# cvxpy/cvxpylayers

Measured on NVIDIA B200. Metric: QP problems/sec fwd+bwd (batch=4096, n=100, m=200, zero+nonneg cones), higher is better.
Workload: dtype f64

## Files before the change

cvxpylayers_b200/_lib.py:

```python
from __future__ import annotations

import ctypes as C
import os
from pathlib import Path

_PKG = Path(__file__).resolve().parent
LIB_PATH = Path(os.environ["BCONE_LIB"]) if os.environ.get("BCONE_LIB") else _PKG / "libbcone.so"

_i32p = C.POINTER(C.c_int32)
_f64p = C.POINTER(C.c_double)

EXPORTS = [
    "bcone_default_settings", "bcone_create", "bcone_destroy", "bcone_last_error", "bcone_set_boundary", "bcone_set_boundary_quad",
    "bcone_ingest", "bcone_emit", "bcone_ingest_pitched", "bcone_emit_pitched", "bcone_peer_alloc", "bcone_peer_open", "bcone_peer_close",
    "bcone_peer_free", "bcone_copy2d_async", "bcone_rows_from_param", "bcone_param_from_rows", "bcone_gather_cols", "bcone_scatter_cols", "bcone_set_param_maps", "bcone_ingest_params", "bcone_emit_params", "bcone_solve", "bcone_solve_warm", "bcone_solve_cached", "bcone_cache_bytes", "bcone_vjp", "bcone_launch_count", "bcone_fallback_count", "bcone_kernel_info", "bcone_path_info", "bcone_memcpy2d", "bcone_set_profile",
]


class BconeDesc(C.Structure):
    _fields_ = [("n", C.c_int32), ("m", C.c_int32), ("nnzA", C.c_int32), ("nnzP", C.c_int32),
                ("A_indptr", _i32p), ("A_indices", _i32p), ("P_indptr", _i32p), ("P_indices", _i32p),
                ("z", C.c_int32), ("l", C.c_int32), ("nq", C.c_int32), ("ns", C.c_int32),
                ("ep", C.c_int32), ("ed", C.c_int32), ("q", _i32p), ("s", _i32p),
                ("device", C.c_int32), ("max_batch", C.c_int32)]


class BconeSettings(C.Structure):
    _fields_ = [("eps_abs", C.c_double), ("eps_rel", C.c_double), ("eps_infeas", C.c_double),
                ("alpha", C.c_double), ("rho_x", C.c_double), ("scale", C.c_double),
                ("lsqr_atol", C.c_double), ("lsqr_btol", C.c_double), ("lsqr_conlim", C.c_double),
                ("max_iters", C.c_int32), ("normalize", C.c_int32), ("adaptive_scale", C.c_int32),
                ("check_interval", C.c_int32), ("ruiz_passes", C.c_int32), ("lsqr_iter_lim", C.c_int32),
                ("lsqr_precond", C.c_int32), ("adaptive_check", C.c_int32),
                ("acceleration_lookback", C.c_int32), ("acceleration_interval", C.c_int32)]


class EngineUnavailable(RuntimeError):
    """libbcone.so is missing / cannot be loaded. There is deliberately no fallback."""


_lib = None


def load() -> C.CDLL:
    global _lib
    if _lib is not None:
        return _lib
    if not LIB_PATH.exists():
        raise EngineUnavailable(
            f"{LIB_PATH} not found: build it with `python -m cvxpylayers_b200.build` (nvcc, sm_100a). "
            "The engine has no CPU or PyTorch fallback.")
    try:
        lib = C.CDLL(str(LIB_PATH))
    except OSError as e:
        raise EngineUnavailable(f"cannot load {LIB_PATH}: {e}") from e
    vp = C.c_void_p
    lib.bcone_default_settings.argtypes = [C.POINTER(BconeSettings)]
    lib.bcone_default_settings.restype = None
    lib.bcone_create.argtypes = [C.POINTER(BconeDesc), C.POINTER(vp)]
    lib.bcone_create.restype = C.c_int
    lib.bcone_destroy.argtypes = [vp]
    lib.bcone_destroy.restype = None
    lib.bcone_last_error.argtypes = [vp]
    lib.bcone_last_error.restype = C.c_char_p
    lib.bcone_set_boundary.argtypes = [vp, C.c_int32, _i32p, C.c_int32, _i32p]
    lib.bcone_set_boundary.restype = C.c_int
    lib.bcone_set_boundary_quad.argtypes = [vp, C.c_int32, _i32p]
    lib.bcone_set_boundary_quad.restype = C.c_int
    lib.bcone_ingest.argtypes = [vp, C.c_int32] + [vp] * 8
    lib.bcone_ingest.restype = C.c_int
    lib.bcone_emit.argtypes = [vp, C.c_int32] + [vp] * 8
    lib.bcone_emit.restype = C.c_int
    lib.bcone_ingest_pitched.argtypes = [vp, C.c_int32, C.c_int64] + [vp] * 8
    lib.bcone_ingest_pitched.restype = C.c_int
    lib.bcone_emit_pitched.argtypes = [vp, C.c_int32, C.c_int64] + [vp] * 8
    lib.bcone_emit_pitched.restype = C.c_int
    lib.bcone_peer_alloc.argtypes = [C.c_int32, C.c_int64, C.POINTER(vp), vp]
    lib.bcone_peer_alloc.restype = C.c_int
    lib.bcone_peer_open.argtypes = [C.c_int32, vp, C.POINTER(vp)]
    lib.bcone_peer_open.restype = C.c_int
    lib.bcone_peer_close.argtypes = [vp]
    lib.bcone_peer_close.restype = C.c_int
    lib.bcone_peer_free.argtypes = [vp]
    lib.bcone_peer_free.restype = C.c_int
    lib.bcone_copy2d_async.argtypes = [vp, C.c_int64, vp, C.c_int64, C.c_int64, C.c_int64, vp]
    lib.bcone_copy2d_async.restype = C.c_int
    lib.bcone_rows_from_param.argtypes = [vp, C.c_int64, vp, C.c_int32, C.c_int32, C.c_int32, vp, vp]
    lib.bcone_rows_from_param.restype = C.c_int
    lib.bcone_param_from_rows.argtypes = [vp, vp, C.c_int64, vp, C.c_int32, C.c_int32, C.c_int32, vp, vp]
    lib.bcone_param_from_rows.restype = C.c_int
    lib.bcone_gather_cols.argtypes = [vp, C.c_int64, vp, vp, C.c_int32, C.c_int32, C.c_int32, vp, vp]
    lib.bcone_gather_cols.restype = C.c_int
    lib.bcone_scatter_cols.argtypes = [vp, vp, C.c_int64, vp, vp, C.c_int32, C.c_int32, C.c_int32, vp, vp]
    lib.bcone_scatter_cols.restype = C.c_int
    lib.bcone_set_param_maps.argtypes = [vp, C.c_int32] + [_i32p, _i32p, _f64p] * 3
    lib.bcone_set_param_maps.restype = C.c_int
    lib.bcone_ingest_params.argtypes = [vp, C.c_int32] + [vp] * 6
    lib.bcone_ingest_params.restype = C.c_int
    lib.bcone_emit_params.argtypes = [vp, C.c_int32] + [vp] * 6
    lib.bcone_emit_params.restype = C.c_int
    lib.bcone_solve.argtypes = [vp, C.c_int32] + [vp] * 10 + [C.POINTER(BconeSettings), vp]
    lib.bcone_solve.restype = C.c_int
    lib.bcone_solve_warm.argtypes = [vp, C.c_int32] + [vp] * 13 + [C.POINTER(BconeSettings), vp]
    lib.bcone_solve_warm.restype = C.c_int
    lib.bcone_solve_cached.argtypes = [vp, C.c_int32] + [vp] * 13 + [vp, C.c_int32, C.POINTER(BconeSettings), vp]
    lib.bcone_solve_cached.restype = C.c_int
    lib.bcone_cache_bytes.argtypes = [vp, C.c_int32]
    lib.bcone_cache_bytes.restype = C.c_size_t
    lib.bcone_vjp.argtypes = [vp, C.c_int32] + [vp] * 14 + [C.POINTER(BconeSettings), vp]
    lib.bcone_vjp.restype = C.c_int
    lib.bcone_memcpy2d.argtypes = [vp, C.c_int64, vp, C.c_int64, C.c_int64, C.c_int64, C.c_int32, vp]
    lib.bcone_memcpy2d.restype = C.c_int
    lib.bcone_set_profile.argtypes = [vp, C.c_int32, C.POINTER(C.c_uint64)]
    lib.bcone_set_profile.restype = C.c_int
    lib.bcone_launch_count.argtypes = [vp]
    lib.bcone_launch_count.restype = C.c_int64
    lib.bcone_fallback_count.argtypes = [vp, _i32p]
    lib.bcone_fallback_count.restype = C.c_int
    lib.bcone_kernel_info.argtypes = [vp] + [_i32p] * 6
    lib.bcone_kernel_info.restype = C.c_int
    lib.bcone_path_info.argtypes = [vp, _i32p, _i32p]
    lib.bcone_path_info.restype = C.c_int
    _lib = lib
    return lib


def default_settings() -> BconeSettings:
    st = BconeSettings()
    load().bcone_default_settings(C.byref(st))
    return st
```

cvxpylayers_b200/csrc/api.cu:

```cuda
#include <cuda_runtime.h>
#include <algorithm>
#include <cstdio>
#include <cstring>
#include <string>
#include <vector>
#include <cstdlib>
#include "common.cuh"

extern "C" {
size_t bc_fwd_smem_bytes(int n, int m, int nnzA, int threads, int max_psd, int indirect, int ns, int nexp);
size_t bc_fwd_ws_doubles(int n, int m, int with_factor);
cudaError_t bc_fwd_configure(int dense, int indirect, size_t smem, int small_cta);
cudaError_t bc_fwd_occupancy(int dense, int indirect, int threads, size_t smem, int *ctas, int small_cta);
cudaError_t bc_fwd_launch(const FwdArgs *a, int indirect, int grid, int threads, size_t smem, cudaStream_t st, int small_cta);
size_t bc_fwdf_smem_bytes(int n, int m);
int bc_fwdf_threads(void);
size_t bc_fwdf_cache_doubles(int n, int m);
int bc_fwdf_eligible(int n, int m);
cudaError_t bc_fwdf_configure(int n, int m, size_t smem);
cudaError_t bc_fwdf_occupancy(int n, int m, size_t smem, int *ctas);
cudaError_t bc_fwdf_launch(const FwdArgs *a, int grid, size_t smem, cudaStream_t st);
size_t bc_bwd_ws_doubles(int n, int m, int npoly);
size_t bc_bwd_smem_bytes(int n, int m, int npoly, int nnzA, int nnzP_smem, int threads, int max_psd, int psd_total, int nexp, int vec_global);
cudaError_t bc_bwd_configure(int dense, size_t smem, int small_cta);
// ... 557 lines not shown
  CK(cudaSetDevice(h->device), "vjp set device");
  a.ws = nullptr; a.ws_stride = (long long)h->bwd_ws_stride;
  if (h->bwd_vec_global && !h->fast_bwd) {
    Handle::StreamWs *sw = stream_ws(h, st);
    if (!ensure_slab(h, &sw->bwd, nullptr, h->bwd_ws_stride * (size_t)h->num_sms * std::max(h->bwd_ctas, h->bwd_ctas_small))) return fail(h, BCONE_ENOMEM, "cudaMalloc backward workspace");
    a.ws = sw->bwd;
  }
  a.inst_list = nullptr; a.B_dev = nullptr; a.fail_list = nullptr; a.fail_count = nullptr; a.prof = h->prof;
  if (h->block_bwd && stg->lsqr_precond == 2) {
    if (h->fail_cap[slot] < B) {
      int *p = nullptr;
      CK(cudaMalloc((void **)&p, (size_t)B * sizeof(int)), "vjp fail list");
      h->allocs.push_back(p); h->fail_list[slot] = p; h->fail_cap[slot] = B;
    }
    CK(cudaMemsetAsync(ctr + 1, 0, 3 * sizeof(int), st), "vjp counters");
    h->last_block_slot = slot;
    a.fail_list = h->fail_list[slot]; a.fail_count = ctr + 2;
    CK(bc_bwdb_launch(&a, std::min(B, h->num_sms), h->blk_threads, h->blk_smem, st), "vjp launch (block)");
    BwdArgs f = a;
    f.st.lsqr_precond = 1; f.counter = ctr + 3; f.inst_list = h->fail_list[slot]; f.B_dev = ctr + 2;
    f.fail_list = nullptr; f.fail_count = nullptr;
    CK(bc_bwdf_launch(&f, std::min(B, h->num_sms * h->bwd_ctas), h->bwd_threads, h->bwd_smem, st), "vjp launch (fallback)");
    h->launches += 2;
    return BCONE_OK;
  }
  if (a.st.lsqr_precond == 2) a.st.lsqr_precond = 1;
  CK(cudaMemsetAsync(ctr + 1, 0, sizeof(int), st), "vjp counter");
  const int use_small = h->bwd_small && (h->small_mode == 2 || B > h->num_sms * h->bwd_ctas);
  const int grid = std::min(B, h->num_sms * (use_small ? h->bwd_ctas_small : h->bwd_ctas));
  if (h->fast_bwd) CK(bc_bwdf_launch(&a, grid, h->bwd_threads, h->bwd_smem, st), "vjp launch (fast)");
  else CK(bc_bwd_launch(&a, grid, h->bwd_threads, h->bwd_smem, st, use_small), "vjp launch");
  h->launches++;
  return BCONE_OK;
}

extern "C" int bcone_memcpy2d(void *dst, int64_t dpitch, const void *src, int64_t spitch, int64_t width, int64_t height,
                              int32_t to_device, void *stream) {
  cudaError_t e = cudaMemcpy2DAsync(dst, (size_t)dpitch, src, (size_t)spitch, (size_t)width, (size_t)height,
                                    to_device ? cudaMemcpyHostToDevice : cudaMemcpyDeviceToHost, (cudaStream_t)stream);
  if (e != cudaSuccess) { g_create_err = std::string("bcone_memcpy2d: ") + cudaGetErrorString(e); return BCONE_ECUDA; }
  return BCONE_OK;
}

extern "C" int bcone_set_profile(void *handle, int32_t on, uint64_t *out) {
  Handle *h = (Handle *)handle;
  if (!h) return BCONE_EINVAL;
  cudaSetDevice(h->device);
  if (out && h->prof) { cudaDeviceSynchronize(); cudaMemcpy(out, h->prof, 32 * sizeof(uint64_t), cudaMemcpyDeviceToHost); cudaMemset(h->prof, 0, 32 * sizeof(uint64_t)); }
  if (on && !h->prof) { if (cudaMalloc((void **)&h->prof, 32 * sizeof(uint64_t)) != cudaSuccess) return BCONE_ENOMEM; h->allocs.push_back(h->prof); cudaMemset(h->prof, 0, 32 * sizeof(uint64_t)); }
  if (!on) h->prof = nullptr;
  return BCONE_OK;
}

extern "C" int bcone_fallback_count(void *handle, int32_t *out) {
  Handle *h = (Handle *)handle;
  if (!h || !out) return BCONE_EINVAL;
  *out = -1;
  if (h->last_block_slot < 0) return BCONE_OK;
  cudaSetDevice(h->device);
  if (cudaDeviceSynchronize() != cudaSuccess) return BCONE_ECUDA;
  int v = 0;
  if (cudaMemcpy(&v, h->counters + 4 * h->last_block_slot + 2, sizeof(int), cudaMemcpyDeviceToHost) != cudaSuccess) return BCONE_ECUDA;
  *out = v;
  return BCONE_OK;
}

extern "C" int64_t bcone_launch_count(void *handle) { return handle ? ((Handle *)handle)->launches : 0; }

extern "C" int bcone_path_info(void *handle, int32_t *fwd_path, int32_t *bwd_path) {
  Handle *h = (Handle *)handle;
  if (!h) return BCONE_EINVAL;
  if (fwd_path) *fwd_path = h->fast_fwd ? 2 : (h->fwd_indirect ? 1 : (h->fwd_factor_global ? 3 : 0));
  if (bwd_path) *bwd_path = h->block_bwd ? 2 : (h->fast_bwd ? 1 : 0);
  return BCONE_OK;
}

extern "C" int bcone_kernel_info(void *handle, int32_t *ft, int32_t *fs, int32_t *fc, int32_t *bt, int32_t *bs, int32_t *bcx) {
  Handle *h = (Handle *)handle;
  if (!h) return BCONE_EINVAL;
  if (ft) *ft = h->fwd_threads; if (fs) *fs = (int32_t)h->fwd_smem; if (fc) *fc = h->fwd_ctas;
  if (bt) *bt = h->bwd_threads; if (bs) *bs = (int32_t)h->bwd_smem; if (bcx) *bcx = h->bwd_ctas;
  return BCONE_OK;
}
```

cvxpylayers_b200/csrc/common.cuh:

```cuda
#pragma once
#include <cuda_runtime.h>
#include <stdint.h>
#include "../../include/bcone.h"

#define BC_TAU_FACTOR 10.0
#define BC_ZERO_CONE_FACTOR 1000.0
#define BC_MIN_SCALE 1e-4
#define BC_MAX_SCALE 1e4
#define BC_RESCALE_MIN_ITERS 100
#define BC_EQ_MIN 1e-4
#define BC_EQ_MAX 1e4

enum { BC_CZERO = 0, BC_CNONNEG = 1, BC_CSOC = 2, BC_CPSD = 3 };

struct DevStruct {
  int n, m, nnzA, nnzP;
  int z, l, nq, ns;
  int ep, ed, exp_start;
  int dense;
  int ncones;
  int max_psd;
  const int *A_indptr, *A_indices;
  const int *At_colptr, *At_rowidx, *At_perm;
  const int *A_rowof;
// ... 513 lines not shown
}

template <bool SQ = false, class Epi>
__device__ __forceinline__ void csr_rows(const double *__restrict__ vals, const int *__restrict__ indptr,
                                         const int *__restrict__ indices, int nrows,
                                         const double *x, Epi ep) {
  constexpr int G = 4;
  const int g = threadIdx.x % G, grp = threadIdx.x / G, ngrp = blockDim.x / G;
  for (int base = 0; base < nrows; base += ngrp) {
    const int i = base + grp;
    double a = 0;
    if (i < nrows) {
      const int e = __ldg(indptr + i + 1);
      for (int k = __ldg(indptr + i) + g; k < e; k += G) { const double q = vals[k]; a = fma(SQ ? q * q : q, x[__ldg(indices + k)], a); }
    }
    a += __shfl_xor_sync(0xffffffffu, a, 1);
    a += __shfl_xor_sync(0xffffffffu, a, 2);
    if (g == 0 && i < nrows) ep(i, a);
  }
}
template <bool SQ = false, class Epi>
__device__ __forceinline__ void csr_cols(const double *__restrict__ vals, const int *__restrict__ colptr,
                                         const int *__restrict__ rowidx, const int *__restrict__ perm, int ncols,
                                         const double *y, Epi ep) {
  constexpr int G = 4;
  const int g = threadIdx.x % G, grp = threadIdx.x / G, ngrp = blockDim.x / G;
  for (int base = 0; base < ncols; base += ngrp) {
    const int j = base + grp;
    double a = 0;
    if (j < ncols) {
      const int e = __ldg(colptr + j + 1);
      for (int k = __ldg(colptr + j) + g; k < e; k += G) { const double q = vals[__ldg(perm + k)]; a = fma(SQ ? q * q : q, y[__ldg(rowidx + k)], a); }
    }
    a += __shfl_xor_sync(0xffffffffu, a, 1);
    a += __shfl_xor_sync(0xffffffffu, a, 2);
    if (g == 0 && j < ncols) ep(j, a);
  }
}

template <bool DENSE, bool SQ = false, class Epi>
__device__ __forceinline__ void A_mul(const DevStruct &S, const double *Av, const double *x, Epi ep, bool wide = false) {
  if (DENSE && wide) dense_rows2<SQ>(Av, S.m, S.n, x, ep);
  else if (DENSE) matvec_rows<SQ>(Av, DenseLayout{S.n}, S.m, S.n, x, ep);
  else csr_rows<SQ>(Av, S.A_indptr, S.A_indices, S.m, x, ep);
}
template <bool DENSE, bool SQ = false, class Epi>
__device__ __forceinline__ void AT_mul(const DevStruct &S, const double *Av, const double *y, double *part, Epi ep, const ColPlan &plA,
                                       bool wide = false) {
  if (DENSE && wide) dense_cols2<SQ>(Av, S.m, S.n, y, part, ep);
  else if (DENSE) matvec_cols<SQ>(Av, DenseLayout{S.n}, S.m, S.n, y, part, ep, plA);
  else { csr_cols<SQ>(Av, S.At_colptr, S.At_rowidx, S.At_perm, S.n, y, ep); __syncthreads(); }
}

template <bool SQ = false, class Epi>
__device__ __forceinline__ void P_mul(const DevStruct &S, const double *Pv, const double *x, double *part, Epi ep, const ColPlan &plN) {
  const int n = S.n;
  if (S.p_dense) {
    matvec_rows<SQ>(Pv, PackedUpperLayout<false>{n}, n, n, x, ep);
    __syncthreads();
    matvec_cols<SQ>(Pv, PackedUpperLayout<true>{n}, n, n, x, part, ep, plN);
  } else {
    csr_rows<SQ>(Pv, S.P_indptr, S.P_indices, n, x, ep);
    __syncthreads();
    constexpr int G = 4;
    const int g = threadIdx.x % G, grp = threadIdx.x / G, ngrp = blockDim.x / G;
    for (int base = 0; base < n; base += ngrp) {
      const int j = base + grp;
      double a = 0;
      if (j < n) {
        const int e = __ldg(S.Pt_colptr + j + 1);
        for (int k = __ldg(S.Pt_colptr + j) + g; k < e; k += G) {
          const int i = __ldg(S.Pt_rowidx + k);
          if (i != j) { const double q = Pv[__ldg(S.Pt_perm + k)]; a = fma(SQ ? q * q : q, x[i], a); }
        }
      }
      a += __shfl_xor_sync(0xffffffffu, a, 1);
      a += __shfl_xor_sync(0xffffffffu, a, 2);
      if (g == 0 && j < n) ep(j, a);
    }
    __syncthreads();
  }
}

__host__ __device__ __forceinline__ int chol_scratch_doubles(int n) { return 26 * ((n + 3) >> 2) + 2; }
__device__ __forceinline__ double rsqrt_nr(double x) {
  double y;
  asm("rsqrt.approx.ftz.f64 %0, %1;" : "=d"(y) : "d"(x));
  double e = fma(-x * y, y, 1.0);
  y = fma(0.5 * y, e, y);
  e = fma(-x * y, y, 1.0);
  return fma(0.5 * y, e, y);
}
struct Tri4 { double l00, l10, l11, l20, l21, l22, l30, l31, l32, l33, m00, m10, m11, m20, m21, m22, m30, m31, m32, m33; bool pd; };
__device__ __forceinline__ Tri4 tri4_block(const double *K, int r0, int jb) {
  Tri4 q;
  const double *R0 = K + ((r0 * (r0 + 1)) >> 1) + r0;
  const double *R1 = K + (((r0 + 1) * (r0 + 2)) >> 1) + r0, *R2 = K + (((r0 + 2) * (r0 + 3)) >> 1) + r0, *R3 = K + (((r0 + 3) * (r0 + 4)) >> 1) + r0;
  const double d00 = R0[0];
  const double d10 = jb > 1 ? R1[0] : 0.0, d11 = jb > 1 ? R1[1] : 1.0;
  const double d20 = jb > 2 ? R2[0] : 0.0, d21 = jb > 2 ? R2[1] : 0.0, d22 = jb > 2 ? R2[2] : 1.0;
  const double d30 = jb > 3 ? R3[0] : 0.0, d31 = jb > 3 ? R3[1] : 0.0, d32 = jb > 3 ? R3[2] : 0.0, d33 = jb > 3 ? R3[3] : 1.0;
  const double p0 = d00, r0_ = rsqrt_nr(p0);
  q.l00 = p0 * r0_; q.l10 = d10 * r0_; q.l20 = d20 * r0_; q.l30 = d30 * r0_;
  const double p1 = fma(-q.l10, q.l10, d11), r1_ = rsqrt_nr(p1);
  q.l11 = p1 * r1_; q.l21 = fma(-q.l20, q.l10, d21) * r1_; q.l31 = fma(-q.l30, q.l10, d31) * r1_;
  const double p2 = fma(-q.l21, q.l21, fma(-q.l20, q.l20, d22)), r2_ = rsqrt_nr(p2);
  q.l22 = p2 * r2_; q.l32 = fma(-q.l31, q.l21, fma(-q.l30, q.l20, d32)) * r2_;
  const double p3 = fma(-q.l32, q.l32, fma(-q.l31, q.l31, fma(-q.l30, q.l30, d33))), r3_ = rsqrt_nr(p3);
  q.l33 = p3 * r3_;
  q.pd = (p0 > 0) && (p1 > 0) && (p2 > 0) && (p3 > 0);
  q.m00 = r0_; q.m11 = r1_; q.m22 = r2_; q.m33 = r3_;
  q.m10 = -q.l10 * q.m00 * r1_;
  q.m20 = -fma(q.l21, q.m10, q.l20 * q.m00) * r2_; q.m21 = -q.l21 * q.m11 * r2_;
  q.m30 = -fma(q.l32, q.m20, fma(q.l31, q.m10, q.l30 * q.m00)) * r3_;
  q.m31 = -fma(q.l32, q.m21, q.l31 * q.m11) * r3_; q.m32 = -q.l32 * q.m22 * r3_;
  return q;
}
#ifdef BC_CHOLPROF
#define CP_STAMP(k) if (prof && t == 0) { const long long now_ = clock64(); atomicAdd(prof + (k), (unsigned long long)(now_ - tt)); tt = now_; }
#else
#define CP_STAMP(k)
#endif
__device__ inline bool chol_inv_packed(double *K, int n, double *tmp, unsigned long long *prof = nullptr) {
  const int T = blockDim.x, t = threadIdx.x, lane = t & 31, warp = t >> 5, nw = T >> 5;
  const int nblk = (n + 3) >> 2, ld = 4 * nblk;
  double *isd = tmp, *moff = tmp + 4 * nblk, *Tst = tmp + 10 * nblk, *flag = tmp + 26 * nblk;
  long long t0 = 0;
  if (prof && t == 0) t0 = clock64();
#ifdef BC_CHOLPROF
  long long tt = t0;
#endif
  const int fr = lane >> 2, fc = lane & 3;
  auto diag_block = [&](int J0) {
    const int jb = min(4, n - J0);
    const Tri4 q = tri4_block(K, J0, jb);
    __syncwarp();
    if (lane == 0) {
      double *D0 = K + ((J0 * (J0 + 1)) >> 1) + J0;
      D0[0] = q.l00;
      if (jb > 1) { double *D1 = K + (((J0 + 1) * (J0 + 2)) >> 1) + J0; D1[0] = q.l10; D1[1] = q.l11; }
      if (jb > 2) { double *D2 = K + (((J0 + 2) * (J0 + 3)) >> 1) + J0; D2[0] = q.l20; D2[1] = q.l21; D2[2] = q.l22; }
      if (jb > 3) { double *D3 = K + (((J0 + 3) * (J0 + 4)) >> 1) + J0; D3[0] = q.l30; D3[1] = q.l31; D3[2] = q.l32; D3[3] = q.l33; }
      isd[J0] = q.m00; isd[J0 + 1] = q.m11; isd[J0 + 2] = q.m22; isd[J0 + 3] = q.m33;
      double *mo = moff + 6 * (J0 >> 2);
      mo[0] = q.m10; mo[1] = q.m20; mo[2] = q.m21; mo[3] = q.m30; mo[4] = q.m31; mo[5] = q.m32;
      if (!q.pd) *flag = 0.0;
    }
  };
  auto trail_tile = [&](int ta, int tb, int J0, int jb, int R0) {
    const int ra = R0 + 8 * ta + fr, rb = R0 + 8 * tb + fr;
    const double fa = (ra < n && fc < jb) ? -K[((ra * (ra + 1)) >> 1) + J0 + fc] : 0.0;
    const double fb = (rb < n && fc < jb) ? K[((rb * (rb + 1)) >> 1) + J0 + fc] : 0.0;
    const int cc = R0 + 8 * tb + 2 * fc;
    double *pc = K + ((ra * (ra + 1)) >> 1) + cc;
    const bool ok0 = ra < n && cc <= ra, ok1 = ra < n && cc + 1 <= ra;
    double c0 = ok0 ? pc[0] : 0.0, c1 = ok1 ? pc[1] : 0.0;
    dmma884(c0, c1, fa, fb);
    if (ok0) pc[0] = c0;
    if (ok1) pc[1] = c1;
  };
  auto inv_tile = [&](int jt, int I0, int ib) {
    double c0 = 0.0, c1 = 0.0, d0 = 0.0, d1 = 0.0;
    const bool zr = fr < ib;
    const double *zrow = K + (((I0 + (zr ? fr : 0)) * (I0 + (zr ? fr : 0) + 1)) >> 1);
    const int jcol = 8 * jt + fr;
    int k = 8 * jt;
    for (int q = 0; q < 2 && k < I0; q++, k += 4) {
      const int k0 = k + fc;
      const double a0 = zr ? zrow[k0] : 0.0;
      const double b0 = jcol <= k0 ? K[((k0 * (k0 + 1)) >> 1) + jcol] : 0.0;
      if (q == 0) dmma884(c0, c1, a0, b0); else dmma884(d0, d1, a0, b0);
    }
    int k0 = k + fc, o0 = ((k0 * (k0 + 1)) >> 1) + jcol;
    for (; k + 8 <= I0; k += 8) {
      const int o1 = o0 + 4 * k0 + 10;
      const double a0 = zr ? zrow[k0] : 0.0, a1 = zr ? zrow[k0 + 4] : 0.0;
      const double b0 = K[o0], b1 = K[o1];
      dmma884(c0, c1, a0, b0);
      dmma884(d0, d1, a1, b1);
      o0 += 8 * k0 + 36; k0 += 8;
    }
    if (k < I0) {
      const double a0 = zr ? zrow[k0] : 0.0;
      dmma884(c0, c1, a0, K[o0]);
    }
    if (fr < 4) {
      const int col = 8 * jt + 2 * fc;
      Tst[fr * ld + col] = c0 + d0; Tst[fr * ld + col + 1] = c1 + d1;
    }
  };
  auto store_X = [&](int I0) {
    const int ib = min(4, n - I0);
    for (int j = (t + (T >> 1)) % T; j < I0; j += T) {
      K[((I0 * (I0 + 1)) >> 1) + j] = Tst[j];
      if (ib > 1) K[(((I0 + 1) * (I0 + 2)) >> 1) + j] = Tst[ld + j];
      if (ib > 2) K[(((I0 + 2) * (I0 + 3)) >> 1) + j] = Tst[2 * ld + j];
      if (ib > 3) K[(((I0 + 3) * (I0 + 4)) >> 1) + j] = Tst[3 * ld + j];
    }
    if (t == T - 1) {
      const double *mo = moff + 6 * (I0 >> 2);
      double *D0 = K + ((I0 * (I0 + 1)) >> 1) + I0;
      D0[0] = isd[I0];
      if (ib > 1) { double *D1 = K + (((I0 + 1) * (I0 + 2)) >> 1) + I0; D1[0] = mo[0]; D1[1] = isd[I0 + 1]; }
      if (ib > 2) { double *D2 = K + (((I0 + 2) * (I0 + 3)) >> 1) + I0; D2[0] = mo[1]; D2[1] = mo[2]; D2[2] = isd[I0 + 2]; }
      if (ib > 3) { double *D3 = K + (((I0 + 3) * (I0 + 4)) >> 1) + I0; D3[0] = mo[3]; D3[1] = mo[4]; D3[2] = mo[5]; D3[3] = isd[I0 + 3]; }
    }
  };
  if (warp == 0) {
    if (lane == 0) *flag = 1.0;
    __syncwarp();
    diag_block(0);
  }
  __syncthreads();
  for (int J0 = 0; J0 < n; J0 += 4) {
    const int jb = min(4, n - J0), R0 = J0 + jb;
    if (*flag == 0.0) return false;
    if (J0 > 0) store_X(J0 - 4);
    const int tz = (t + T - (T >> 2)) % T;
    if (R0 + t < n || tz < J0) {
      const double *mo = moff + 6 * (J0 >> 2);
      const double m00 = isd[J0], m11 = isd[J0 + 1], m22 = isd[J0 + 2], m33 = isd[J0 + 3];
      const double m10 = mo[0], m20 = mo[1], m21 = mo[2], m30 = mo[3], m31 = mo[4], m32 = mo[5];
      for (int i = R0 + t; i < n; i += T) {
        double *row = K + ((i * (i + 1)) >> 1) + J0;
        const double a0 = row[0], a1 = jb > 1 ? row[1] : 0.0, a2 = jb > 2 ? row[2] : 0.0, a3 = jb > 3 ? row[3] : 0.0;
        row[0] = a0 * m00;
        if (jb > 1) row[1] = fma(a1, m11, a0 * m10);
        if (jb > 2) row[2] = fma(a2, m22, fma(a1, m21, a0 * m20));
        if (jb > 3) row[3] = fma(a3, m33, fma(a2, m32, fma(a1, m31, a0 * m30)));
      }
      double *L0 = K + ((J0 * (J0 + 1)) >> 1), *L1 = K + (((J0 + 1) * (J0 + 2)) >> 1), *L2 = K + (((J0 + 2) * (J0 + 3)) >> 1),
             *L3 = K + (((J0 + 3) * (J0 + 4)) >> 1);
      for (int i = tz; i < J0; i += T) {
        const double a0 = L0[i], a1 = jb > 1 ? L1[i] : 0.0, a2 = jb > 2 ? L2[i] : 0.0, a3 = jb > 3 ? L3[i] : 0.0;
        L0[i] = -(m00 * a0);
        if (jb > 1) L1[i] = -fma(m11, a1, m10 * a0);
        if (jb > 2) L2[i] = -fma(m22, a2, fma(m21, a1, m20 * a0));
        if (jb > 3) L3[i] = -fma(m33, a3, fma(m32, a2, fma(m31, a1, m30 * a0)));
      }
    }
    CP_STAMP(17);
    __syncthreads();
    CP_STAMP(18);
    {
      const int ntl = R0 < n ? (n - R0 + 7) >> 3 : 0, ntile = (ntl * (ntl + 1)) >> 1;
      const int ntj = (J0 + 7) >> 3;
      if (warp == 0 && ntile > 0) {
        trail_tile(0, 0, J0, jb, R0);
        __syncwarp();
        diag_block(R0);
      }
      if (warp > 0 || nw == 1) {
        const int W = nw > 1 ? nw - 1 : 1, w0 = nw > 1 ? warp - 1 : 0;
        const int nwork = ntj + (ntile > 0 ? ntile - 1 : 0);
        int ta = 0, tb = 0, e_cur = 0;
        for (int u = w0; u < nwork; u += W) {
          if (u < ntj) inv_tile(u, J0, jb);
          else {
            const int e = u - ntj + 1;
            tb += e - e_cur; e_cur = e;
            while (tb > ta) { tb -= ta + 1; ta++; }
            trail_tile(ta, tb, J0, jb, R0);
          }
        }
      }
    }
    CP_STAMP(19);
    __syncthreads();
    CP_STAMP(20);
  }
  if (*flag == 0.0) return false;
  store_X(((n - 1) >> 2) << 2);
  __syncthreads();
  if (prof && t == 0) { const long long t1 = clock64(); atomicAdd(prof + 5, (unsigned long long)(t1 - t0)); }
  return true;
}

__device__ void jacobi_eig_warp(int k, double *X, double *V);

__device__ __forceinline__ void project_soc_warp(double *v, int sz) {
  const int lane = threadIdx.x & 31;
  if (sz == 1) { if (lane == 0 && v[0] < 0) v[0] = 0; return; }
  double ss = 0;
  for (int i = 1 + lane; i < sz; i += 32) ss += v[i] * v[i];
  ss = warp_sum(ss);
  const double nx = sqrt(ss), t = v[0];
  __syncwarp();
  if (nx <= t) return;
  if (nx <= -t) { for (int i = lane; i < sz; i += 32) v[i] = 0; return; }
  const double a = 0.5 * (1.0 + t / nx);
  for (int i = 1 + lane; i < sz; i += 32) v[i] *= a;
  if (lane == 0) v[0] = a * nx;
}

__device__ __forceinline__ void svec_to_mat_warp(int k, const double *v, double *X) {
  const int lane = threadIdx.x & 31;
  const double is2 = 0.70710678118654752440;
  for (int e = lane; e < k * k; e += 32) {
    int i = e / k, j = e % k;
    int r = max(i, j), c = min(i, j);
    int idx = c * k - (c * (c - 1)) / 2 + (r - c);
    X[e] = (i == j) ? v[idx] : v[idx] * is2;
  }
}
__device__ __forceinline__ void mat_to_svec_warp(int k, const double *X, double *v) {
  const int lane = threadIdx.x & 31;
  const double s2 = 1.41421356237309504880;
  for (int e = lane; e < k * k; e += 32) {
    int i = e / k, j = e % k;
    if (i < j) continue;
    int idx = j * k - (j * (j - 1)) / 2 + (i - j);
    v[idx] = (i == j) ? X[i * k + i] : 0.5 * (X[i * k + j] + X[j * k + i]) * s2;
  }
}

__device__ inline void jacobi_eig_warp(int k, double *X, double *V) {
  const int lane = threadIdx.x & 31;
  for (int e = lane; e < k * k; e += 32) V[e] = (e / k == e % k) ? 1.0 : 0.0;
  __syncwarp();
  for (int sweep = 0; sweep < 30; sweep++) {
    int rotations = 0;
    for (int p = 0; p < k - 1; p++) for (int q = p + 1; q < k; q++) {
      const double apq = X[p * k + q];
      if (fabs(apq) <= 1e-17 * (fabs(X[p * k + p]) + fabs(X[q * k + q])) || apq == 0.0) continue;
      rotations++;
      const double app = X[p * k + p], aqq = X[q * k + q];
      const double theta = (aqq - app) / (2.0 * apq);
      const double t = (theta >= 0 ? 1.0 : -1.0) / (fabs(theta) + sqrt(theta * theta + 1.0));
      const double c = 1.0 / sqrt(t * t + 1.0), s = t * c;
      __syncwarp();
      for (int r = lane; r < k; r += 32) {
        double xp = X[r * k + p], xq = X[r * k + q];
        X[r * k + p] = c * xp - s * xq; X[r * k + q] = s * xp + c * xq;
        double vp = V[r * k + p], vq = V[r * k + q];
        V[r * k + p] = c * vp - s * vq; V[r * k + q] = s * vp + c * vq;
      }
      __syncwarp();
      for (int r = lane; r < k; r += 32) {
        double xp = X[p * k + r], xq = X[q * k + r];
        X[p * k + r] = c * xp - s * xq; X[q * k + r] = s * xp + c * xq;
      }
      __syncwarp();
    }
    if (rotations == 0) break;
  }
  __syncwarp();
}

template <class FA, class FB, class ST>
__device__ __forceinline__ void warp_mm16(int k, FA fa, FB fb, ST st) {
  const int lane = threadIdx.x & 31, fr = lane >> 2, fc = lane & 3;
  const int nt = (k + 7) >> 3, nk = (k + 3) >> 2;
  for (int ti = 0; ti < nt; ti++) {
    double d[2][2] = {{0.0, 0.0}, {0.0, 0.0}};
    for (int ks = 0; ks < nk; ks++) {
      const double a = fa(8 * ti + fr, 4 * ks + fc);
// ... 305 lines not shown
```

include/bcone.h:

```cpp
#ifndef BCONE_H
#define BCONE_H
#include <stdint.h>

#ifdef __cplusplus
extern "C" {
#endif

typedef struct {
  int32_t n, m, nnzA, nnzP;
  const int32_t *A_indptr, *A_indices;
  const int32_t *P_indptr, *P_indices;
  int32_t z, l, nq, ns, ep, ed;
  const int32_t *q, *s;
  int32_t device;
  int32_t max_batch;
} bcone_desc;

typedef struct {
  double eps_abs, eps_rel, eps_infeas;
  double alpha, rho_x, scale;
  double lsqr_atol, lsqr_btol, lsqr_conlim;
  int32_t max_iters, normalize, adaptive_scale, check_interval;
  int32_t ruiz_passes, lsqr_iter_lim;
  int32_t lsqr_precond;
  int32_t adaptive_check;
  int32_t acceleration_lookback;
  int32_t acceleration_interval;
} bcone_settings;

enum { BCONE_SOLVED = 1, BCONE_INACCURATE = 2, BCONE_UNBOUNDED = -1, BCONE_INFEASIBLE = -2, BCONE_FAILED = -4 };
enum { BCONE_OK = 0, BCONE_EINVAL = -1, BCONE_ECUDA = -2, BCONE_ENOMEM = -3, BCONE_EUNSUPPORTED = -4 };

void bcone_default_settings(bcone_settings *st);

int bcone_create(const bcone_desc *desc, void **handle);
void bcone_destroy(void *handle);
const char *bcone_last_error(void *handle);

int bcone_set_boundary(void *handle, int32_t nnz_aug, const int32_t *gather, int32_t nb, const int32_t *b_idx);
int bcone_set_boundary_quad(void *handle, int32_t nnzP_boundary, const int32_t *gatherP);
int bcone_ingest(void *handle, int32_t B, const double *A_eval, const double *q_eval, const double *P_eval,
                 double *A_vals, double *P_vals, double *b, double *c, void *cuda_stream);
int bcone_emit(void *handle, int32_t B, const double *dA_vals, const double *dP_vals, const double *db,
               const double *dc, double *dA_eval, double *dq_eval, double *dP_eval, void *cuda_stream);

int bcone_ingest_pitched(void *handle, int32_t B, int64_t ldb, const double *A_eval, const double *q_eval, const double *P_eval,
                         double *A_vals, double *P_vals, double *b, double *c, void *cuda_stream);
int bcone_emit_pitched(void *handle, int32_t B, int64_t ldb, const double *dA_vals, const double *dP_vals, const double *db,
                       const double *dc, double *dA_eval, double *dq_eval, double *dP_eval, void *cuda_stream);

int bcone_peer_alloc(int32_t device, int64_t bytes, void **ptr, void *ipc_handle64);
int bcone_peer_open(int32_t device, const void *ipc_handle64, void **ptr);
int bcone_peer_close(void *ptr);
int bcone_peer_free(void *ptr);
int bcone_copy2d_async(void *dst, int64_t dpitch, const void *src, int64_t spitch, int64_t width, int64_t height, void *cuda_stream);

int bcone_set_param_maps(void *handle, int32_t P1, const int32_t *A_ptr, const int32_t *A_col, const double *A_val,
                         const int32_t *q_ptr, const int32_t *q_col, const double *q_val,
                         const int32_t *P_ptr, const int32_t *P_col, const double *P_val);
int bcone_ingest_params(void *handle, int32_t B, const double *p_stack, double *A_vals, double *P_vals, double *b,
                        double *c, void *cuda_stream);
int bcone_emit_params(void *handle, int32_t B, const double *dA_vals, const double *dP_vals, const double *db,
                      const double *dc, double *dp_stack, void *cuda_stream);

int bcone_rows_from_param(const double *param, int64_t stride, const int32_t *map, int32_t K, int32_t B, int32_t op, double *rows,
                          void *cuda_stream);
int bcone_param_from_rows(const double *grows, const double *param, int64_t stride, const int32_t *map, int32_t K, int32_t B,
                          int32_t op, double *gparam, void *cuda_stream);
int bcone_gather_cols(const double *in, int64_t ld, const int32_t *map, const double *scale, int32_t K, int32_t B, int32_t op,
                      double *out, void *cuda_stream);
int bcone_scatter_cols(const double *gout, const double *out, int64_t ld, const int32_t *map, const double *scale, int32_t K,
                       int32_t B, int32_t op, double *gin, void *cuda_stream);

int bcone_solve(void *handle, int32_t B, const double *A_vals, const double *P_vals, const double *b,
                const double *c, double *x, double *y, double *s, int32_t *status, int32_t *iters,
                double *resid, const bcone_settings *st, void *cuda_stream);

int bcone_solve_warm(void *handle, int32_t B, const double *A_vals, const double *P_vals, const double *b, const double *c,
                     const double *x0, const double *y0, const double *s0, double *x, double *y, double *s,
                     int32_t *status, int32_t *iters, double *resid, const bcone_settings *st, void *cuda_stream);

size_t bcone_cache_bytes(void *handle, int32_t B);
int bcone_solve_cached(void *handle, int32_t B, const double *A_vals, const double *P_vals, const double *b, const double *c,
                       const double *x0, const double *y0, const double *s0, double *x, double *y, double *s,
                       int32_t *status, int32_t *iters, double *resid, void *cache, int32_t reuse,
                       const bcone_settings *st, void *cuda_stream);

int bcone_vjp(void *handle, int32_t B, const double *A_vals, const double *P_vals, const double *b,
              const double *c, const double *x, const double *y, const double *s, const double *dx,
              const double *dy, double *dA_vals, double *dP_vals, double *db, double *dc,
              int32_t *lsqr_iters, const bcone_settings *st, void *cuda_stream);

int bcone_memcpy2d(void *dst, int64_t dpitch, const void *src, int64_t spitch, int64_t width, int64_t height,
                   int32_t to_device, void *cuda_stream);

int bcone_set_profile(void *handle, int32_t on, uint64_t *out16);

int64_t bcone_launch_count(void *handle);
int bcone_fallback_count(void *handle, int32_t *out);
int bcone_kernel_info(void *handle, int32_t *fwd_threads, int32_t *fwd_smem, int32_t *fwd_ctas_per_sm,
                      int32_t *bwd_threads, int32_t *bwd_smem, int32_t *bwd_ctas_per_sm);
int bcone_path_info(void *handle, int32_t *fwd_path, int32_t *bwd_path);

#ifdef __cplusplus
}
#endif
#endif
```

Baseline: 284,600.

## Replace interleaved triangular inverse with recursive-doubling blocked inverse after Cholesky

The packed Cholesky-inverse routine no longer builds the inverse of L column-block by column-block inside the factorization loop, which needed extra staging scratch and added work to each step. It now factors first, then inverts L with a recursive-doubling scheme: it writes the diagonal 4x4 inverses, combines adjacent pairs, and then merges blocks of doubling size using DMMA tensor-core tiles in two passes. Scratch shrinks and each factor step gets shorter, at the cost of a separate inverse phase with many block-wide barriers. A debug entry point for testing the routine is also added.

After: 287,800 (median of 6 runs). 1.01x the previous value.

```diff
diff --git a/cvxpylayers_b200/_lib.py b/cvxpylayers_b200/_lib.py
--- a/cvxpylayers_b200/_lib.py
+++ b/cvxpylayers_b200/_lib.py
@@ -13,7 +13,7 @@
 EXPORTS = [
     "bcone_default_settings", "bcone_create", "bcone_destroy", "bcone_last_error", "bcone_set_boundary", "bcone_set_boundary_quad",
     "bcone_ingest", "bcone_emit", "bcone_ingest_pitched", "bcone_emit_pitched", "bcone_peer_alloc", "bcone_peer_open", "bcone_peer_close",
-    "bcone_peer_free", "bcone_copy2d_async", "bcone_rows_from_param", "bcone_param_from_rows", "bcone_gather_cols", "bcone_scatter_cols", "bcone_set_param_maps", "bcone_ingest_params", "bcone_emit_params", "bcone_solve", "bcone_solve_warm", "bcone_solve_cached", "bcone_cache_bytes", "bcone_vjp", "bcone_launch_count", "bcone_fallback_count", "bcone_kernel_info", "bcone_path_info", "bcone_memcpy2d", "bcone_set_profile",
+    "bcone_peer_free", "bcone_copy2d_async", "bcone_rows_from_param", "bcone_param_from_rows", "bcone_gather_cols", "bcone_scatter_cols", "bcone_set_param_maps", "bcone_ingest_params", "bcone_emit_params", "bcone_solve", "bcone_solve_warm", "bcone_solve_cached", "bcone_cache_bytes", "bcone_vjp", "bcone_launch_count", "bcone_fallback_count", "bcone_kernel_info", "bcone_path_info", "bcone_memcpy2d", "bcone_set_profile", "bcone_debug_chol_inv",
 ]
 
 
@@ -113,6 +113,8 @@
     lib.bcone_memcpy2d.restype = C.c_int
     lib.bcone_set_profile.argtypes = [vp, C.c_int32, C.POINTER(C.c_uint64)]
     lib.bcone_set_profile.restype = C.c_int
+    lib.bcone_debug_chol_inv.argtypes = [C.c_int32, C.c_int32, C.c_int32, vp, vp, vp, vp]
+    lib.bcone_debug_chol_inv.restype = C.c_int
     lib.bcone_launch_count.argtypes = [vp]
     lib.bcone_launch_count.restype = C.c_int64
     lib.bcone_fallback_count.argtypes = [vp, _i32p]
diff --git a/cvxpylayers_b200/csrc/api.cu b/cvxpylayers_b200/csrc/api.cu
--- a/cvxpylayers_b200/csrc/api.cu
+++ b/cvxpylayers_b200/csrc/api.cu
@@ -663,3 +663,30 @@
   if (bt) *bt = h->bwd_threads; if (bs) *bs = (int32_t)h->bwd_smem; if (bcx) *bcx = h->bwd_ctas;
   return BCONE_OK;
 }
+
+__global__ void __launch_bounds__(512) debug_chol_kernel(const double *K_in, double *out, int32_t *ok, int n, int on_chip) {
+  extern __shared__ __align__(16) double dsm[];
+  const int np = (n * (n + 1)) >> 1;
+  const double *src = K_in + (size_t)blockIdx.x * np;
+  double *dst = out + (size_t)blockIdx.x * np;
+  double *K = on_chip ? dsm : dst, *tmp = on_chip ? dsm + ((np + 1) & ~1) : dsm;
+  for (int k = threadIdx.x; k < np; k += blockDim.x) K[k] = src[k];
+  __syncthreads();
+  const bool pd = chol_inv_packed(K, n, tmp);
+  if (on_chip)
+    for (int k = threadIdx.x; k < np; k += blockDim.x) dst[k] = K[k];
+  if (threadIdx.x == 0) ok[blockIdx.x] = pd;
+}
+
+extern "C" int bcone_debug_chol_inv(int32_t n, int32_t threads, int32_t B, const double *K_in, double *out, int32_t *ok, void *stream) {
+  if (n < 1 || n > 512 || threads < 64 || threads > 512 || threads % 32 || B < 1 || !K_in || !out || !ok) return BCONE_EINVAL;
+  const int on_chip = n <= 128;
+  const size_t smem = sizeof(double) * ((on_chip ? (((n * (n + 1)) / 2 + 1) & ~1) : 0) + chol_scratch_doubles(n));
+  cudaError_t e = cudaFuncSetAttribute(debug_chol_kernel, cudaFuncAttributeMaxDynamicSharedMemorySize, (int)smem);
+  if (e == cudaSuccess) {
+    debug_chol_kernel<<<B, threads, smem, (cudaStream_t)stream>>>(K_in, out, ok, n, on_chip);
+    e = cudaGetLastError();
+  }
+  if (e != cudaSuccess) { g_create_err = std::string("bcone_debug_chol_inv: ") + cudaGetErrorString(e); return BCONE_ECUDA; }
+  return BCONE_OK;
+}
diff --git a/cvxpylayers_b200/csrc/common.cuh b/cvxpylayers_b200/csrc/common.cuh
--- a/cvxpylayers_b200/csrc/common.cuh
+++ b/cvxpylayers_b200/csrc/common.cuh
@@ -619,7 +619,7 @@
   }
 }
 
-__host__ __device__ __forceinline__ int chol_scratch_doubles(int n) { return 26 * ((n + 3) >> 2) + 2; }
+__host__ __device__ __forceinline__ int chol_scratch_doubles(int n) { return 10 * ((n + 3) >> 2) + 2; }
 __device__ __forceinline__ double rsqrt_nr(double x) {
   double y;
   asm("rsqrt.approx.ftz.f64 %0, %1;" : "=d"(y) : "d"(x));
@@ -654,19 +654,18 @@
   return q;
 }
 #ifdef BC_CHOLPROF
-#define CP_STAMP(k) if (prof && t == 0) { const long long now_ = clock64(); atomicAdd(prof + (k), (unsigned long long)(now_ - tt)); tt = now_; }
+#define CP_MARK() const long long cp_mark_ = clock64()
+#define CP_MAX(s, k) if (prof && lane == 0) atomicMax(prof + 64 + 4 * (s) + (k), (unsigned long long)(clock64() - cp_mark_))
 #else
-#define CP_STAMP(k)
+#define CP_MARK()
+#define CP_MAX(s, k)
 #endif
 __device__ inline bool chol_inv_packed(double *K, int n, double *tmp, unsigned long long *prof = nullptr) {
   const int T = blockDim.x, t = threadIdx.x, lane = t & 31, warp = t >> 5, nw = T >> 5;
-  const int nblk = (n + 3) >> 2, ld = 4 * nblk;
-  double *isd = tmp, *moff = tmp + 4 * nblk, *Tst = tmp + 10 * nblk, *flag = tmp + 26 * nblk;
+  const int nblk = (n + 3) >> 2;
+  double *isd = tmp, *moff = tmp + 4 * nblk, *flag = tmp + 10 * nblk;
   long long t0 = 0;
   if (prof && t == 0) t0 = clock64();
-#ifdef BC_CHOLPROF
-  long long tt = t0;
-#endif
   const int fr = lane >> 2, fc = lane & 3;
   auto diag_block = [&](int J0) {
     const int jb = min(4, n - J0);
@@ -696,53 +695,7 @@
     if (ok0) pc[0] = c0;
     if (ok1) pc[1] = c1;
   };
-  auto inv_tile = [&](int jt, int I0, int ib) {
-    double c0 = 0.0, c1 = 0.0, d0 = 0.0, d1 = 0.0;
-    const bool zr = fr < ib;
-    const double *zrow = K + (((I0 + (zr ? fr : 0)) * (I0 + (zr ? fr : 0) + 1)) >> 1);
-    const int jcol = 8 * jt + fr;
-    int k = 8 * jt;
-    for (int q = 0; q < 2 && k < I0; q++, k += 4) {
-      const int k0 = k + fc;
-      const double a0 = zr ? zrow[k0] : 0.0;
-      const double b0 = jcol <= k0 ? K[((k0 * (k0 + 1)) >> 1) + jcol] : 0.0;
-      if (q == 0) dmma884(c0, c1, a0, b0); else dmma884(d0, d1, a0, b0);
-    }
-    int k0 = k + fc, o0 = ((k0 * (k0 + 1)) >> 1) + jcol;
-    for (; k + 8 <= I0; k += 8) {
-      const int o1 = o0 + 4 * k0 + 10;
-      const double a0 = zr ? zrow[k0] : 0.0, a1 = zr ? zrow[k0 + 4] : 0.0;
-      const double b0 = K[o0], b1 = K[o1];
-      dmma884(c0, c1, a0, b0);
-      dmma884(d0, d1, a1, b1);
-      o0 += 8 * k0 + 36; k0 += 8;
-    }
-    if (k < I0) {
-      const double a0 = zr ? zrow[k0] : 0.0;
-      dmma884(c0, c1, a0, K[o0]);
-    }
-    if (fr < 4) {
-      const int col = 8 * jt + 2 * fc;
-      Tst[fr * ld + col] = c0 + d0; Tst[fr * ld + col + 1] = c1 + d1;
-    }
-  };
-  auto store_X = [&](int I0) {
-    const int ib = min(4, n - I0);
-    for (int j = (t + (T >> 1)) % T; j < I0; j += T) {
-      K[((I0 * (I0 + 1)) >> 1) + j] = Tst[j];
-      if (ib > 1) K[(((I0 + 1) * (I0 + 2)) >> 1) + j] = Tst[ld + j];
-      if (ib > 2) K[(((I0 + 2) * (I0 + 3)) >> 1) + j] = Tst[2 * ld + j];
-      if (ib > 3) K[(((I0 + 3) * (I0 + 4)) >> 1) + j] = Tst[3 * ld + j];
-    }
-    if (t == T - 1) {
-      const double *mo = moff + 6 * (I0 >> 2);
-      double *D0 = K + ((I0 * (I0 + 1)) >> 1) + I0;
-      D0[0] = isd[I0];
-      if (ib > 1) { double *D1 = K + (((I0 + 1) * (I0 + 2)) >> 1) + I0; D1[0] = mo[0]; D1[1] = isd[I0 + 1]; }
-      if (ib > 2) { double *D2 = K + (((I0 + 2) * (I0 + 3)) >> 1) + I0; D2[0] = mo[1]; D2[1] = mo[2]; D2[2] = isd[I0 + 2]; }
-      if (ib > 3) { double *D3 = K + (((I0 + 3) * (I0 + 4)) >> 1) + I0; D3[0] = mo[3]; D3[1] = mo[4]; D3[2] = mo[5]; D3[3] = isd[I0 + 3]; }
-    }
-  };
+  auto minv = [&](int r0, int a, int b) { return a == b ? isd[r0 + a] : moff[6 * (r0 >> 2) + ((a * (a - 1)) >> 1) + b]; };
   if (warp == 0) {
     if (lane == 0) *flag = 1.0;
     __syncwarp();
@@ -752,63 +705,137 @@
   for (int J0 = 0; J0 < n; J0 += 4) {
     const int jb = min(4, n - J0), R0 = J0 + jb;
     if (*flag == 0.0) return false;
-    if (J0 > 0) store_X(J0 - 4);
-    const int tz = (t + T - (T >> 2)) % T;
-    if (R0 + t < n || tz < J0) {
-      const double *mo = moff + 6 * (J0 >> 2);
-      const double m00 = isd[J0], m11 = isd[J0 + 1], m22 = isd[J0 + 2], m33 = isd[J0 + 3];
-      const double m10 = mo[0], m20 = mo[1], m21 = mo[2], m30 = mo[3], m31 = mo[4], m32 = mo[5];
-      for (int i = R0 + t; i < n; i += T) {
-        double *row = K + ((i * (i + 1)) >> 1) + J0;
-        const double a0 = row[0], a1 = jb > 1 ? row[1] : 0.0, a2 = jb > 2 ? row[2] : 0.0, a3 = jb > 3 ? row[3] : 0.0;
-        row[0] = a0 * m00;
-        if (jb > 1) row[1] = fma(a1, m11, a0 * m10);
-        if (jb > 2) row[2] = fma(a2, m22, fma(a1, m21, a0 * m20));
-        if (jb > 3) row[3] = fma(a3, m33, fma(a2, m32, fma(a1, m31, a0 * m30)));
-      }
-      double *L0 = K + ((J0 * (J0 + 1)) >> 1), *L1 = K + (((J0 + 1) * (J0 + 2)) >> 1), *L2 = K + (((J0 + 2) * (J0 + 3)) >> 1),
-             *L3 = K + (((J0 + 3) * (J0 + 4)) >> 1);
-      for (int i = tz; i < J0; i += T) {
-        const double a0 = L0[i], a1 = jb > 1 ? L1[i] : 0.0, a2 = jb > 2 ? L2[i] : 0.0, a3 = jb > 3 ? L3[i] : 0.0;
-        L0[i] = -(m00 * a0);
-        if (jb > 1) L1[i] = -fma(m11, a1, m10 * a0);
-        if (jb > 2) L2[i] = -fma(m22, a2, fma(m21, a1, m20 * a0));
-        if (jb > 3) L3[i] = -fma(m33, a3, fma(m32, a2, fma(m31, a1, m30 * a0)));
-      }
-    }
-    CP_STAMP(17);
+    if (R0 >= n) break;
+#ifdef BC_CHOLPROF
+    const long long cp_step_ = clock64();
+#endif
+    {
+      CP_MARK();
+      if (R0 + t < n) {
+        const double *mo = moff + 6 * (J0 >> 2);
+        const double m00 = isd[J0], m11 = isd[J0 + 1], m22 = isd[J0 + 2], m33 = isd[J0 + 3];
+        const double m10 = mo[0], m20 = mo[1], m21 = mo[2], m30 = mo[3], m31 = mo[4], m32 = mo[5];
+        for (int i = R0 + t; i < n; i += T) {
+          double *row = K + ((i * (i + 1)) >> 1) + J0;
+          const double a0 = row[0], a1 = row[1], a2 = row[2], a3 = row[3];
+          row[0] = a0 * m00;
+          row[1] = fma(a1, m11, a0 * m10);
+          row[2] = fma(a2, m22, fma(a1, m21, a0 * m20));
+          row[3] = fma(a3, m33, fma(a2, m32, fma(a1, m31, a0 * m30)));
+        }
+      }
+      CP_MAX(J0 >> 2, 0);
+    }
     __syncthreads();
-    CP_STAMP(18);
+    CP_MARK();
     {
-      const int ntl = R0 < n ? (n - R0 + 7) >> 3 : 0, ntile = (ntl * (ntl + 1)) >> 1;
-      const int ntj = (J0 + 7) >> 3;
-      if (warp == 0 && ntile > 0) {
-        trail_tile(0, 0, J0, jb, R0);
+      const int ntl = (n - R0 + 7) >> 3, ntile = (ntl * (ntl + 1)) >> 1;
+      if (warp == 0) {
+        trail_tile(0, 0, J0, 4, R0);
         __syncwarp();
         diag_block(R0);
-      }
-      if (warp > 0 || nw == 1) {
-        const int W = nw > 1 ? nw - 1 : 1, w0 = nw > 1 ? warp - 1 : 0;
-        const int nwork = ntj + (ntile > 0 ? ntile - 1 : 0);
+        CP_MAX(J0 >> 2, 1);
+      } else {
         int ta = 0, tb = 0, e_cur = 0;
-        for (int u = w0; u < nwork; u += W) {
-          if (u < ntj) inv_tile(u, J0, jb);
-          else {
-            const int e = u - ntj + 1;
-            tb += e - e_cur; e_cur = e;
-            while (tb > ta) { tb -= ta + 1; ta++; }
-            trail_tile(ta, tb, J0, jb, R0);
+        for (int e = warp; e < ntile; e += nw - 1) {
+          tb += e - e_cur; e_cur = e;
+          while (tb > ta) { tb -= ta + 1; ta++; }
+          trail_tile(ta, tb, J0, 4, R0);
+        }
+        CP_MAX(J0 >> 2, 2);
+      }
+    }
+    __syncthreads();
+#ifdef BC_CHOLPROF
+    if (prof && t == 0) prof[64 + J0 + 3] = clock64() - cp_step_;
+#endif
+  }
+#ifdef BC_CHOLPROF
+  const long long cp_inv_ = clock64();
+#endif
+  for (int e = t; e < 16 * nblk; e += T) {
+    const int r0 = 4 * (e >> 4), a = (e >> 2) & 3, b = e & 3;
+    if (b <= a && r0 + a < n) K[(((r0 + a) * (r0 + a + 1)) >> 1) + r0 + b] = minv(r0, a, b);
+  }
+  {
+    const int ne = 16 * ((n + 3) >> 3);
+    int base = 0;
+    do {
+      const int e = base + t, p = e >> 4, i = (e >> 2) & 3, j = e & 3, r1 = 8 * p, r2 = r1 + 4;
+      const bool live = e < ne && r2 + i < n;
+      double v = 0.0;
+      if (live) {
+        for (int k = 0; k <= i; k++) {
+          const double *Lk = K + (((r2 + k) * (r2 + k + 1)) >> 1) + r1;
+          double w = 0.0;
+          for (int l = j; l < 4; l++) w = fma(Lk[l], minv(r1, l, j), w);
+          v = fma(minv(r2, i, k), w, v);
+        }
+      }
+      __syncthreads();
+      if (live) K[(((r2 + i) * (r2 + i + 1)) >> 1) + r1 + j] = -v;
+      __syncthreads();
+      base += T;
+    } while (base < ne);
+  }
+  constexpr int MAXT = 4;
+  for (int b = 8; b < n; b <<= 1) {
+    const int nc = b >> 3, strip = ((n + b - 1) / (2 * b)) * nc, ntile = strip * nc;
+    for (int pass = 0; pass < 2; pass++) {
+      for (int base = 0; base < ntile; base += MAXT * nw) {
+        double c[MAXT][2];
+#pragma unroll
+        for (int q = 0; q < MAXT; q++) {
+          const int u = base + warp + q * nw, hi = u / strip, p = (u % strip) / nc, lo = u % nc;
+          const int it = pass ? nc - 1 - hi : lo, jt = pass ? lo : hi, r1 = 2 * b * p, r2 = r1 + b;
+          double c0 = 0.0, c1 = 0.0, d0 = 0.0, d1 = 0.0;
+          if (u < ntile && r2 + 8 * it < n) {
+            const int ia = 8 * it + fr, ra = r2 + ia;
+            const bool rok = ra < n;
+            if (pass == 0) {
+              const int col = 8 * jt + fr;
+              const double *Lrow = K + ((ra * (ra + 1)) >> 1) + r1;
+              for (int k = 8 * jt; k < b; k += 8) {
+                const int ka = k + fc, kb = k + 4 + fc;
+                const double a0 = rok ? Lrow[ka] : 0.0, a1 = rok ? Lrow[kb] : 0.0;
+                const double b0 = ka >= col ? K[(((r1 + ka) * (r1 + ka + 1)) >> 1) + r1 + col] : 0.0;
+                const double b1 = kb >= col ? K[(((r1 + kb) * (r1 + kb + 1)) >> 1) + r1 + col] : 0.0;
+                dmma884(c0, c1, a0, b0);
+                dmma884(d0, d1, a1, b1);
+              }
+            } else {
+              const int col = r1 + 8 * jt + fr;
+              const double *Xrow = K + ((ra * (ra + 1)) >> 1) + r2;
+              for (int k = 0; k < 8 * it + 8; k += 8) {
+                const int ka = k + fc, kb = k + 4 + fc;
+                const double a0 = rok && ka <= ia ? Xrow[ka] : 0.0, a1 = rok && kb <= ia ? Xrow[kb] : 0.0;
+                const double b0 = r2 + ka < n ? K[(((r2 + ka) * (r2 + ka + 1)) >> 1) + col] : 0.0;
+                const double b1 = r2 + kb < n ? K[(((r2 + kb) * (r2 + kb + 1)) >> 1) + col] : 0.0;
+                dmma884(c0, c1, a0, b0);
+                dmma884(d0, d1, a1, b1);
+              }
+            }
+          }
+          c[q][0] = c0 + d0; c[q][1] = c1 + d1;
+        }
+        __syncthreads();
+        const double sgn = pass ? -1.0 : 1.0;
+#pragma unroll
+        for (int q = 0; q < MAXT; q++) {
+          const int u = base + warp + q * nw, hi = u / strip, p = (u % strip) / nc, lo = u % nc;
+          const int it = pass ? nc - 1 - hi : lo, jt = pass ? lo : hi, r1 = 2 * b * p, ra = r1 + b + 8 * it + fr;
+          if (u < ntile && ra < n) {
+            double *pc = K + ((ra * (ra + 1)) >> 1) + r1 + 8 * jt + 2 * fc;
+            pc[0] = sgn * c[q][0]; pc[1] = sgn * c[q][1];
           }
         }
-      }
-    }
-    CP_STAMP(19);
-    __syncthreads();
-    CP_STAMP(20);
-  }
-  if (*flag == 0.0) return false;
-  store_X(((n - 1) >> 2) << 2);
-  __syncthreads();
+        __syncthreads();
+      }
+    }
+  }
+#ifdef BC_CHOLPROF
+  if (prof && t == 0) prof[62] = clock64() - cp_inv_;
+#endif
   if (prof && t == 0) { const long long t1 = clock64(); atomicAdd(prof + 5, (unsigned long long)(t1 - t0)); }
   return true;
 }
diff --git a/include/bcone.h b/include/bcone.h
--- a/include/bcone.h
+++ b/include/bcone.h
@@ -96,6 +96,8 @@
 
 int bcone_set_profile(void *handle, int32_t on, uint64_t *out16);
 
+int bcone_debug_chol_inv(int32_t n, int32_t threads, int32_t B, const double *K_in, double *out, int32_t *ok, void *cuda_stream);
+
 int64_t bcone_launch_count(void *handle);
 int bcone_fallback_count(void *handle, int32_t *out);
 int bcone_kernel_info(void *handle, int32_t *fwd_threads, int32_t *fwd_smem, int32_t *fwd_ctas_per_sm,
```
